# joelle-o-world/dusp

Hardware: AMD Instinct MI355X
Metric: rendered Msamples/sec (whole node) + HBM GB/s fraction, 1024-voice 48kHz (higher is better)
Workload: dtype f64; 1 GPU; configs[2] per-voice: 1024 voices/GPU x Multiply(Osc(10k), Ramp(T,1,0) triggered), 60s @48000 Hz, every voice's PCM written; voices_per_gpu=1024, voices_total=1024, n_samples=2880000, engine=fused, parallelism=voices sharded over 1 GPU(s), no collective

## Files before the change

### dusp_amd/csrc/abi_context.hip

```cpp
#include <cmath>
#include <cstdio>
#include <cstdlib>
#include <cstring>
#include <memory>

#include "abi_internal.hpp"
#include "device_util.hpp"
#include "jit_engine.hpp"
#include "table_checks.hpp"

thread_local std::string g_error;

static dusp::Knobs read_knobs() {
    dusp::Knobs k;
    auto num = [](const char *name, int fallback) {
        const char *e = getenv(name);
        return e && *e ? atoi(e) : fallback;
    };
    if (const char *t = getenv("DUSP_FUSED_TABLE")) k.fused_table_global = t[0] == 'g';
    k.fused_R = num("DUSP_FUSED_R", k.fused_R);
    k.fused_items = num("DUSP_FUSED_ITEMS", k.fused_items);
    k.fused_fx32 = num("DUSP_FUSED_FX32", k.fused_fx32);
    k.fused_segmajor = num("DUSP_FUSED_SEGMAJOR", k.fused_segmajor);
    k.wave_segments = num("DUSP_WAVE_SEGMENTS", k.wave_segments);
    k.wave_max_waves = num("DUSP_WAVE_MAX_WAVES", k.wave_max_waves);
    k.wave_jit = num("DUSP_WAVE_JIT", k.wave_jit);
    k.wave_per_wave = num("DUSP_WAVE_PER_WAVE", k.wave_per_wave);
    k.jit_profile = num("DUSP_JIT_PROFILE", k.jit_profile);
    k.filter_fma = num("DUSP_FILTER_FMA", k.filter_fma);
    k.jit_spill_bytes = num("DUSP_JIT_SPILL", k.jit_spill_bytes);
    k.jit_lds_table = num("DUSP_JIT_LDS_TABLE", k.jit_lds_table);
    k.jit_lean = num("DUSP_JIT_LEAN", k.jit_lean);
    k.jit_log = num("DUSP_JIT_LOG", k.jit_log);
    k.ring_window = num("DUSP_RING_WINDOW", k.ring_window);
    k.filter_scan = num("DUSP_FILTER_SCAN", k.filter_scan);
    k.filter_warm = num("DUSP_FILTER_WARM", k.filter_warm);
    k.jit_nt = num("DUSP_JIT_NT", k.jit_nt);
    k.delay_line = num("DUSP_DELAY_LINE", k.delay_line);
    k.jit_rotate = num("DUSP_JIT_ROTATE", k.jit_rotate);
    k.ring_poison = num("DUSP_RING_POISON", k.ring_poison);
    k.mix_width = num("DUSP_MIX_WIDTH", k.mix_width);
    k.mix_depth = num("DUSP_MIX_DEPTH", k.mix_depth);
    k.mix_tile_mb = num("DUSP_MIX_TILE_MB", k.mix_tile_mb);
    k.score_plan_kb = num("DUSP_SCORE_PLAN_KB", k.score_plan_kb);
    if (const char *f = getenv("DUSP_JIT_FORCE")) {
        int w = 0, r = 0;
        if (std::sscanf(f, "%dx%d", &w, &r) == 2 && w >= 1 && w <= 16 && r >= 1 && r <= 4) k.jit_force_waves = w, k.jit_force_per_wave = r;
    }
    return k;
}

extern "C" {

const char *dusp_version(void) { return "dusp-hip 0.1.0 (gfx950)"; }
int dusp_abi_version(void) { return DUSP_ABI_VERSION; }

// ... 197 lines not shown
```

### dusp_amd/csrc/abi_internal.hpp

```cpp
#pragma once
#include <limits>
#include <cmath>
#include <hip/hip_runtime.h>

#include <algorithm>
#include <cstddef>
#include <cstdint>
#include <exception>
#include <map>
#include <mutex>
#include <new>
#include <stdexcept>
#include <string>
#include <utility>
#include <vector>

#include "../../include/dusp_hip.h"
#include "device_types.hpp"
#include "fused_plan.hpp"
#include "jit_codegen.hpp"
#include "program.hpp"
#include "score_plan.hpp"

namespace dusp {
// ... 148 lines not shown
        f("staging parameters", d_host_par);
        f("staging inputs", d_host_in);
        f("hand-off buffers", d_handoff_init);
        f("hand-off buffers", d_handoff_out);
        f("program constants", d_ops);
        f("program constants", d_out_bufs);
        f("program constants", d_init);
        f("compiled kernel's constants", d_jit_fk);
        f("compiled kernel's constants", d_jit_dk);
        f("compiled kernel's constants", d_jit_scan);
        f("warm-up records", d_warm_records);
        f("warm-up start state", d_warm_init);
        f("column verdicts", d_jit_regime);
    }
    const char *first_overwritten() {
        const char *hit = nullptr;
        for_each_workspace([&](const char *name, auto &buf) {
            if (!hit && !buf.intact()) hit = name;
        });
        return hit;
    }
};
static_assert(sizeof(dusp_workspaces) == dusp_workspaces::kCount * sizeof(DevBuf<char>), "dusp_workspaces holds DevBufs only: update kCount and for_each_workspace");

struct dusp_program : dusp_workspaces {
    dusp_ctx *ctx = nullptr;
    dusp::Program P;
    int engine = DUSP_ENGINE_CHUNK;
    dusp::FusedPlan fused;
    dusp::WavePlan wave;
    std::vector<dusp::SumVoice> h_sum_voices;
    std::vector<double> h_sum_end;
    uint32_t last_n_inst = 0, last_n_pad = 0;
    bool rendered = false;
    std::vector<double> h_state;
    bool h_state_valid = false;
    bool mixed = false;
    std::vector<unsigned> mix_range;
    uint32_t mix_n_inst = 0;
    int requested_engine = DUSP_ENGINE_AUTO;
    bool resumable = false;
    bool persistent = false;
    bool keep_memory = false;
    bool delay_changed = false;
    bool migrate_to_chunk = false;
    int64_t next_clock = 0;
    hipEvent_t ev0 = nullptr, ev1 = nullptr;
    hipStream_t last_stream = nullptr;
    bool jit_ok = false;
    std::string jit_why;
    std::map<std::pair<int, int>, dusp::JitSource> jit_src;
    bool jit_consts_uploaded = false;
    int voice_loop = -1;
    uint64_t jit_table_generation = 0;
    int jit_waves = 0, jit_per_wave = 0;
    unsigned jit_segments = 1;
    unsigned wave_segments = 1;
    std::vector<double> param_bound;
    bool jit_voices = false;
    bool jit_scan = false;
    bool handoff_ok = false;
    std::string handoff_why;
    unsigned warm_redo_from = 0;
    unsigned char *pin[1] = {nullptr};
    size_t pin_bytes = 0;

// ... 135 lines not shown
```

### dusp_amd/csrc/abi_program.hip

```cpp
#include <cmath>
#include <cstdio>
#include <cstdlib>
#include <cstring>
#include <memory>

#include "abi_internal.hpp"
#include "engine_select.hpp"
#include "jit_engine.hpp"

extern "C" {

static int select_engine(dusp_program *prog) {
    dusp_ctx *ctx = prog->ctx;
    dusp::EngineRequest rq;
    rq.requested = prog->requested_engine;
    rq.resumable = prog->resumable;
    rq.rendered = prog->rendered;
    rq.engine_so_far = prog->engine;
    rq.delay_changed = prog->delay_changed;
    rq.wave_jit = ctx->knobs.wave_jit;
    for (int k = 0; k < dusp::kNumTables; k++) rq.table_set[k] = ctx->table_set[k], rq.table_fx32_ok[k] = ctx->table_fx32_ok[k];
    dusp::EngineChoice choice = dusp::engine_select(prog->P, rq, std::move(prog->wave.ramp_checked));
    prog->fused = std::move(choice.fused);
    prog->wave = std::move(choice.wave);
// ... 133 lines not shown
        prog->requested_engine = before.engine;
        const int back = finish_build(prog);
        prog->requested_engine = requested;
        ctx->err = back == DUSP_OK ? why : why + " (and the previous program could not be restored: " + ctx->err + ")";
        return rc;
    }
    prog->keep_memory = persistent;
    if (persistent && engine_before == DUSP_ENGINE_WAVE && prog->engine == DUSP_ENGINE_CHUNK) prog->migrate_to_chunk = true;
    return DUSP_OK;
    });
}

void dusp_program_destroy(dusp_program *prog) {
    if (!prog) return;
    (void)hipSetDevice(prog->ctx->device);
    if (prog->rendered && prog->ev1) (void)hipEventSynchronize(prog->ev1);
    (void)hipStreamSynchronize(prog->ctx->stream);
    delete prog;
}

int dusp_program_info_get(const dusp_program *prog, dusp_program_info *info) {
    if (!prog || !info) return DUSP_ERR_ARG;
    std::memset(info, 0, sizeof *info);
    const dusp::Graph &g = prog->P.g;
    info->sample_rate = (uint32_t)g.sample_rate;
    info->chunk_size = (uint32_t)g.chunk;
    info->n_units = (uint32_t)g.units.size();
    info->n_out_channels = (uint32_t)prog->P.out_bufs.size();
    info->n_params = (uint32_t)g.n_params;
    info->engine = (uint32_t)prog->engine;
    info->n_device_ops = (uint32_t)prog->P.ops.size();
    info->n_inputs = (uint32_t)g.n_inputs;
    if (prog->engine == DUSP_ENGINE_FUSED) std::snprintf(info->shape, sizeof info->shape, "%s", prog->fused.shape.c_str());
    if (prog->engine == DUSP_ENGINE_WAVE && prog->jit_ok && (prog->jit_waves || !prog->rendered))
    {
        const int at = std::snprintf(info->shape, sizeof info->shape, "%s, compiled kernel: %d units, %dx%d", prog->P.feed_forward ? "feed-forward" : "feedback",
                                     (int)prog->P.ops.size(), prog->jit_waves, prog->jit_per_wave);
        if (at > 0 && (size_t)at < sizeof info->shape && (prog->jit_voices || prog->jit_segments > 1)) {
            if (prog->jit_voices && prog->jit_segments > 1) std::snprintf(info->shape + at, sizeof info->shape - (size_t)at, ", loop, %u seg", prog->jit_segments);
            else if (prog->jit_voices) std::snprintf(info->shape + at, sizeof info->shape - (size_t)at, ", voice loop");
            else if (prog->warm_redo_from) std::snprintf(info->shape + at, sizeof info->shape - (size_t)at, ", %u seg, redo@%u", prog->jit_segments, prog->warm_redo_from);
            else std::snprintf(info->shape + at, sizeof info->shape - (size_t)at, ", %u seg", prog->jit_segments);
        } else if (at > 0 && (size_t)at < sizeof info->shape && prog->jit_scan)
            std::snprintf(info->shape + at, sizeof info->shape - (size_t)at, ", scan");
    }
    else if (prog->engine == DUSP_ENGINE_WAVE && prog->jit_ok)
        std::snprintf(info->shape, sizeof info->shape, "%s, %d chunk buffers in LDS (kernel compiling)", prog->P.feed_forward ? "feed-forward" : "feedback", prog->wave.n_slots);
    else if (prog->engine == DUSP_ENGINE_WAVE && prog->rendered && prog->wave_segments > 1)
        std::snprintf(info->shape, sizeof info->shape, "%s, %d chunk buffers in LDS, %u seg", prog->P.feed_forward ? "feed-forward" : "feedback", prog->wave.n_slots, prog->wave_segments);
    else if (prog->engine == DUSP_ENGINE_WAVE)
        std::snprintf(info->shape, sizeof info->shape, "%s, %d chunk buffers in LDS", prog->P.feed_forward ? "feed-forward" : "feedback", prog->wave.n_slots);
    if (prog->engine == DUSP_ENGINE_CHUNK && !prog->P.warm_ops.empty() && !prog->handoff_ok && !prog->handoff_why.empty())
        std::snprintf(info->shape, sizeof info->shape, "warm-up, then not compiled: %.34s", prog->handoff_why.c_str());
    if (prog->engine == DUSP_ENGINE_CHUNK && prog->handoff_ok && prog->jit_waves)
        std::snprintf(info->shape, sizeof info->shape, "%d warm-up chunks here, then compiled kernel: %d units, %dx%d", (int)prog->P.warm_ops.size(), (int)prog->P.ops.size(),
                      prog->jit_waves, prog->jit_per_wave);
    return DUSP_OK;
}

int dusp_state_download(dusp_program *prog, size_t instance, size_t unit, double *out, size_t cap) {
    if (!prog) return DUSP_ERR_ARG;
    dusp_ctx *ctx = prog->ctx;
    return guarded(ctx->err, "dusp_state_download", [&]() -> int {
    if (!prog->rendered) CTX_FAIL(ctx, DUSP_ERR_STATE, "dusp_state_download: nothing has been rendered yet");
    if (prog->mixed) CTX_FAIL(ctx, DUSP_ERR_STATE, "dusp_state_download: the last render was a mix (dusp_render_host_mix, dusp_render_host_score): unit state describes its last tile only");
    const dusp::Graph &g = prog->P.g;
// ... 138 lines not shown
```

### dusp_amd/csrc/abi_render.hip

```cpp
#include <cstring>

#include "abi_internal.hpp"
#include "jit_plan.hpp"
#include "render_plan.hpp"
#include "ring_windows.hpp"

static int check_tables(dusp_program *prog) {
    dusp_ctx *ctx = prog->ctx;
    for (const auto &u : prog->P.g.units)
        if (u.op == dusp::OP_OSC || u.op == dusp::OP_MULTI_OSC || u.op == dusp::OP_SHAPE) {
            const int w = (int)u.attrs[0];
            if (!ctx->d_tables || !ctx->table_set[w])
                CTX_FAIL(ctx, DUSP_ERR_STATE, "render: wave table " + std::to_string(w) + " has not been uploaded (dusp_table_upload)");
            if (ctx->table_len != (uint32_t)prog->P.g.sample_rate + 1)
                CTX_FAIL(ctx, DUSP_ERR_STATE, "render: wave table length != sample_rate + 1");
        }
    return DUSP_OK;
}


hipError_t zero_rings(dusp_program *prog, uint32_t n_pad, uint32_t n_chunks, bool instance_major, hipStream_t stream) {
    const dusp::Program &P = prog->P;
    float *rings = prog->d_rings.p;
    const size_t total = (size_t)P.ring_samples;
// ... 101 lines not shown
    }
    dusp::build_sum_voices(prog->fused, (uint32_t)prog->P.g.sample_rate, gb, L.chain_first + (uint64_t)c.n_chunks * dusp::kChunk, prog->h_sum_voices, prog->h_sum_end);
    HIP_TRY(ctx, prog->d_sum_voices.ensure(prog->h_sum_voices.size()));
    HIP_TRY(ctx, hipMemcpyAsync(prog->d_sum_voices.p, prog->h_sum_voices.data(), prog->h_sum_voices.size() * sizeof(dusp::SumVoice), hipMemcpyHostToDevice, stream));
    std::vector<double> end((size_t)prog->fused.n_state_words * n_inst);
    for (int w = 0; w < prog->fused.n_state_words; w++)
        for (uint32_t i = 0; i < n_inst; i++) end[(size_t)w * n_inst + i] = prog->h_sum_end[(size_t)w];
    HIP_TRY(ctx, hipMemcpyAsync(prog->d_fused_state.p, end.data(), end.size() * sizeof(double), hipMemcpyHostToDevice, stream));
    HIP_TRY(ctx, hipStreamSynchronize(stream));
    HIP_TRY(ctx, hipEventRecord(prog->ev0, stream));
    HIP_TRY(ctx, dusp::launch_sumchain(prog->fused, L, prog->d_sum_voices.p, gb, stream));
    HIP_TRY(ctx, hipEventRecord(prog->ev1, stream));
    return DUSP_OK;
}

static int render_fused(dusp_program *prog, const RenderCall &c, const ChainWindow *window) {
    dusp_ctx *ctx = prog->ctx;
    dusp::FusedLaunch L{};
    L.params = c.d_params;
    L.tables = ctx->d_tables;
    L.table_stride = ctx->table_stride;
    L.out = c.d_out;
    L.n_inst = c.n_inst;
    L.n_samples = c.n_samples;
    L.n_chunks = c.n_chunks;
    L.sample_rate = (uint32_t)prog->P.g.sample_rate;
    L.n_cus = ctx->n_cus;
    L.table_antisym = ctx->table_antisym[prog->fused.table_id];
    L.table_finite = ctx->table_finite[prog->fused.table_id];
    L.table_fx32_ok = ctx->table_fx32_ok[prog->fused.table_id];
    L.table_delta = ctx->table_delta[prog->fused.table_id];
    L.table_form = ctx->table_form[prog->fused.table_id];
    L.knobs = ctx->knobs;
    HIP_TRY(ctx, prog->d_recs.ensure(c.n_inst));
    L.recs = prog->d_recs.p;
    HIP_TRY(ctx, prog->d_fused_state.ensure((size_t)std::max(1, prog->fused.n_state_words) * c.n_inst));
    L.end_state = prog->d_fused_state.p;
    if (prog->fused.kind == dusp::FUSED_SUMCHAIN) {
        if (int rc = render_sum_chain(prog, c, L, window)) return rc;
    } else {
        HIP_TRY(ctx, hipEventRecord(prog->ev0, c.stream));
        HIP_TRY(ctx, dusp::launch_fused(prog->fused, L, c.stream));
        HIP_TRY(ctx, hipEventRecord(prog->ev1, c.stream));
    }
    finish_render(prog, c.n_inst, c.n_pad, c.n_chunks);
    return DUSP_OK;
}

static int render_wave_interpreter(dusp_program *prog, const RenderCall &c) {
    dusp_ctx *ctx = prog->ctx;
    const dusp::Program &P = prog->P;
    const uint32_t n_inst = c.n_inst, n_pad = c.n_pad, n_chunks = c.n_chunks;
    hipStream_t stream = c.stream;
    HIP_TRY(ctx, prog->d_state.ensure(state_workspace_doubles(P, n_pad)));
    dusp::WaveArgs w{};
    w.ops = prog->d_ops.p;
    w.out_bufs = prog->d_out_bufs.p;
    w.params = c.d_params;
    w.tables = ctx->d_tables;
    w.inputs = c.d_inputs;
    w.out = c.d_out;
    w.state = prog->d_state.p;
    w.init_state = prog->d_init.p;
    w.n_samples = c.n_samples;
    w.n_ops = (uint32_t)P.ops.size();
    w.n_out = (uint32_t)P.out_bufs.size();
    w.n_inst = n_inst;
// ... 202 lines not shown
```

### dusp_amd/csrc/device_types.hpp

```cpp
#pragma once
#if defined(__HIPCC_RTC__)
typedef unsigned int uint32_t;
typedef int int32_t;
typedef unsigned long long uint64_t;
typedef long long int64_t;
typedef unsigned long uintptr_t;
#else
#include <cstdint>
#endif

namespace dusp {

enum : int {
    OP_OSC = 1, OP_RAMP, OP_MULTIPLY, OP_SUM, OP_FILTER, OP_DELAY, OP_CB_READER, OP_CB_WRITER, OP_REPEATER,
    OP_SUBTRACT, OP_DIVIDE, OP_POLARITY_INVERT, OP_ABS, OP_CLIP, OP_HARD_CLIP_ABOVE, OP_HARD_CLIP_BELOW,
    OP_SECONDS_TO_SAMPLES, OP_FIXED_MULTIPLY, OP_GAIN, OP_DECIBEL_TO_SCALER, OP_SEMITONE_TO_RATIO, OP_POW,
    OP_FIXED_DELAY, OP_COMB_FILTER, OP_ALL_PASS, OP_MONO_DELAY, OP_READBACK_DELAY, OP_MULTI_OSC,
    OP_PAN, OP_MIDI_TO_FREQUENCY, OP_RESCALE, OP_CROSS_FADER, OP_VECTOR_MAGNITUDE, OP_TIMER, OP_SAMPLE_RATE_REDUX,
    OP_CONCAT_CHANNELS, OP_PICK_CHANNEL,
    OP_SHAPE, OP_AHD,
    OP_HOST_ONLY,
    OP_INPUT,
    OP_RETRIGGER,
    OP_MAP_FIRST = OP_SUBTRACT, OP_MAP_LAST = OP_POW,
    OP_WIDE_FIRST = OP_PAN, OP_WIDE_LAST = OP_VECTOR_MAGNITUDE
};
constexpr int kMaxIn = 5;
enum : int { IN_CONST = 0, IN_CONNECT = 1, IN_PARAM = 2 };
enum : int { SRC_CONST = 0, SRC_BUF = 1, SRC_PARAM = 2 };
constexpr int kNumTables = 9;
constexpr int kFirstShapeTable = 5;
constexpr int kChunk = 256;
constexpr unsigned long half_table_image_bytes(uint32_t sample_rate) {
    return ((unsigned long)((sample_rate / 2 + 1) + ((sample_rate / 2 + 1) >> 5) + 2) * 4ul + 15ul) & ~15ul;
}
constexpr int kMaxWarmChunks = 8;

struct Knobs {
    int fused_table_global = 0;
    int fused_R = 4;
    int fused_items = 0;
    int fused_fx32 = 1;
    int fused_segmajor = 0;
    int wave_segments = -1;
    int wave_max_waves = 0;
    int wave_jit = 1;
    int wave_per_wave = 0;
    int jit_lean = 1;
    int jit_log = 0;
    int jit_lds_table = 1;
    int jit_spill_bytes = 96;
    int jit_force_waves = 0;
    int jit_force_per_wave = 0;
    int ring_window = 1;
    int ring_poison = 0;
    int filter_scan = 1;
    int filter_warm = 1;
    int jit_nt = 0;
    int jit_rotate = 1;
    int delay_line = 1;
    int filter_fma = 0;
    int jit_profile = 0;
    int mix_width = 0;
    int mix_depth = 0;
    int mix_tile_mb = 0;
    int score_plan_kb = 0;
};

#if defined(__HIPCC__)
typedef float f32x4 __attribute__((ext_vector_type(4)));
#endif

struct DevOperand {
    int32_t kind;
    int32_t idx;
    float cval;
// ... 31 lines not shown
```

### dusp_amd/csrc/fused_engine.hip

```cpp
#include <hip/hip_runtime.h>

#include <type_traits>

#include "device_types.hpp"
#include "fused_device.hpp"
#include "fused_plan.hpp"
#include "repeat_add.hpp"

namespace dusp {

namespace {

template <bool FASTDIV>
__device__ __forceinline__ float ramp_value(const FusedArgs &A, double tn, double dy) {
    const double tt = fmin(tn, A.r_d);
    double q;
    if (FASTDIV) {
        q = tt * A.r_rcp;
        const double rem = fma(-q, A.r_d, tt);
        q = fma(rem, A.r_rcp, q);
    } else
        q = tt / A.r_d;
    return (float)(A.r_y0 + q * dy);
}

__device__ __forceinline__ float shape_value(const FusedArgs &A, double t, double srd) {
    const double l = (double)A.s_min, h = (double)A.s_max;
    if (t <= 0.0) return (float)((A.s_left_is_shape ? (double)A.s_table[0] : A.s_left) * (h - l) + l);
    if (t > srd) return (float)((A.s_right_is_shape ? (double)A.s_table[(uint32_t)srd] : A.s_right) * (h - l) + l);
    if (t != t) return __builtin_nanf("");
    const double fl = floor(t), frac = t - fl;
    return (float)(l + (h - l) * ((double)A.s_table[(int)ceil(t)] * frac + (double)A.s_table[(int)fl] * (1.0 - frac)));
}

__device__ __forceinline__ void start_phase(const OscRec &rc, uint32_t seg, uint32_t lane, uint64_t (&P)[4]) {
    const uint64_t base = addmod(addmod(rc.P0, rc.Fm, rc.S), mulmod(rc.segstep, seg, rc.S), rc.S);
    P[0] = addmod(base, mulmod(rc.step4, lane, rc.S), rc.S);
    for (int c = 1; c < 4; ++c) P[c] = addmod(P[c - 1], rc.Fm, rc.S);
}

}

static __device__ int fused_prepare_voice(const FusedArgs &A, OscRec *recs, const uint32_t inst) {
    const uint32_t sr = A.sample_rate;
    const double srd = (double)sr;
    OscRec rc;
    double fd = (double)operand_value(A.f, A.params, A.n_inst, inst);
    const float f_in = operand_value(A.f, A.params, A.n_inst, inst);
    rc.bad = !(fabs(fd) <= 3.4028234663852886e38);
    if (!rc.bad && osc_const_beyond_exact(f_in, sr)) rc.bad = 2;
    if (rc.bad) fd = 0.0;
    if (fabs(fd) >= srd) fd = fmod(fd, srd);
    int E = 0;
    if (fd != 0.0) E = min(E, lsb_exponent(fd));
    if (A.phase0 != 0.0) E = min(E, lsb_exponent(A.phase0));
    const int Emin = -(62 - (32 - __builtin_clz(sr)));
    if (E < Emin) E = Emin;
    rc.E = E;
    rc.u = ldexp(1.0, E);
    rc.S = (uint64_t)sr << (-E);
    const long long F = (long long)rint(ldexp(fd, -E));
    rc.Fm = F >= 0 ? (uint64_t)F : rc.S - (uint64_t)(-F);
    if (rc.Fm >= rc.S) rc.Fm -= rc.S;
    rc.P0 = (uint64_t)rint(ldexp(A.phase0, -E));
    if (rc.P0 >= rc.S) rc.P0 %= rc.S;
    rc.step4 = mulmod(rc.Fm, 4, rc.S);
    rc.step256 = mulmod(rc.Fm, kChunk, rc.S);
    rc.segstep = mulmod(rc.Fm, (uint64_t)A.seg_groups * kChunk, rc.S);
    rc.gain = A.gain.kind == SRC_PARAM || A.gain.kind == SRC_CONST ? operand_value(A.gain, A.params, A.n_inst, inst) : 1.f;
    rc.pad = 0;
    recs[inst] = rc;
// ... 16 lines not shown
        const double t_end = A.s_playing ? repeat_add(A.s_t0, A.s_c, T_end) : A.s_t0;
        A.end_state[(size_t)A.shape_state_word * A.n_inst + inst] = t_end;
        A.end_state[(size_t)(A.shape_state_word + 1) * A.n_inst + inst] = A.s_playing ? 1.0 : 0.0;
        A.end_state[(size_t)(A.shape_state_word + 2) * A.n_inst + inst] = (A.s_finished || (T_end > 0 && t_end > srd)) ? 1.0 : 0.0;
    }
    return rc.bad;
}

static __device__ void fused_reference_voice(const FusedArgs &A, const OscRec *recs, const uint32_t inst, const uint32_t lane, const int kind) {
    const double srd = (double)A.sample_rate, dy = A.r_y1 - A.r_y0;
    const float f = operand_value(A.f, A.params, A.n_inst, inst), gain = recs[inst].gain;
    float *row = A.out + (size_t)inst * A.n_samples;
    double phase = A.phase0;
    for (uint32_t g = 0; g < A.n_groups; ++g) {
        double mine[4];
        phase = osc_reference_chunk(phase, srd, lane, [&](uint32_t, int) { return f; }, mine);
#pragma unroll
        for (int c = 0; c < 4; ++c) {
            const uint64_t n = (uint64_t)g * kChunk + lane * 4 + c;
            float v = osc_reference_lookup(A.table, mine[c], srd);
            if (kind == FUSED_OSC_RAMP) v = v * ramp_value<false>(A, A.r_playing ? A.r_t0 + (double)(n + 1) : A.r_t0, dy);
            if (kind == FUSED_OSC_SHAPE) v = v * shape_value(A, A.s_playing ? repeat_add(A.s_t0, A.s_c, n + 1) : A.s_t0, srd);
            if (kind == FUSED_OSC_GAIN) v = v * gain;
            if (n < A.n_samples) row[n] = fix_out<false>(v);
        }
    }
}

__global__ void __launch_bounds__(256) dusp_fused_prepare(FusedArgs A, OscRec *recs, int kind) {
    __shared__ uint32_t flagged[256], n_flagged;
    if (threadIdx.x == 0) n_flagged = 0u;
    __syncthreads();
    const uint32_t inst = blockIdx.x * blockDim.x + threadIdx.x;
    if (inst < A.n_inst && fused_prepare_voice(A, recs, inst) == 2) flagged[atomicAdd(&n_flagged, 1u)] = inst;
    __syncthreads();
    for (uint32_t k = threadIdx.x >> 6; k < n_flagged; k += 4u) fused_reference_voice(A, recs, flagged[k], threadIdx.x & 63u, kind);
}

template <int KIND, int TBL, int R, bool FASTDIV, bool FINITE, int BLOCK>
__global__ void __launch_bounds__(BLOCK) dusp_fused_kernel(FusedArgs A, const OscRec *__restrict__ recs) {
    extern __shared__ __attribute__((aligned(16))) float lds_table[];
    Table<TBL> table;
    table.g = A.table;
    table.h = lds_table;
    table.N = A.sample_rate + 1;
    table.M = A.sample_rate / 2;
    table.form = make_table_form(A.table_form, A.sample_rate);
    if (TBL == 1) load_half_table<BLOCK>(lds_table, A.table, A.sample_rate);
    const uint32_t lane = threadIdx.x & 63u;
    constexpr uint32_t waves_per_block = BLOCK / 64;
    constexpr int RS = R < 4 ? R : 4;
    const uint32_t n_blk = (A.n_inst + R - 1) / R;
    const uint64_t n_items = (uint64_t)n_blk * A.n_seg;
    const uint64_t total_waves = (uint64_t)gridDim.x * waves_per_block;
    const double srd = (double)A.sample_rate;
    const uint32_t sr = A.sample_rate;
    const double dy = A.r_y1 - A.r_y0;
    const uint32_t n_full = A.vec4_ok ? (uint32_t)(A.n_samples / kChunk) : 0u;

    for (uint64_t item = (uint64_t)blockIdx.x * waves_per_block + (threadIdx.x >> 6); item < n_items; item += total_waves) {
        const uint32_t blk = A.seg_major ? (uint32_t)(item / A.n_seg) : (uint32_t)(item % n_blk);
        const uint32_t seg = A.seg_major ? (uint32_t)(item % A.n_seg) : (uint32_t)(item / n_blk);
        const uint32_t g0 = seg * A.seg_groups;
        const uint32_t g1 = min(g0 + A.seg_groups, A.n_groups);
        const uint32_t gm = max(g0, min(g1, n_full));
        const uint64_t t_start = (uint64_t)g0 * kChunk;

        uint32_t inst[R];
        int e_min = 0;
        bool any_bad = false;
#pragma unroll
        for (int r = 0; r < R; ++r) {
            inst[r] = min(blk * R + r, A.n_inst - 1);
            e_min = min(e_min, recs[inst[r]].E);
            any_bad = any_bad || recs[inst[r]].bad;
        }
        float *const row0 = A.out + t_start + lane * 4;
        const double tn0 = A.r_t0 + (A.r_playing ? (double)(t_start + lane * 4 + 1) : 0.0);
        const double tn_step = A.r_playing ? (double)kChunk : 0.0;
        const double tn_c = A.r_playing ? 1.0 : 0.0;
        double tn;
        const double st0 = (KIND == FUSED_OSC_SHAPE && A.s_playing) ? repeat_add(A.s_t0, A.s_c, t_start) : A.s_t0;
        double st;
        auto ramp4 = [&](float (&rv)[4]) {
            if (KIND == FUSED_OSC_SHAPE) {
                if (!A.s_playing) {
#pragma unroll
                    for (int c = 0; c < 4; ++c) rv[c] = shape_value(A, st, srd);
                } else {
                    long long T, ce;
                    int K;
                    if (linear_run(st, A.s_c, kChunk, T, ce, K)) {
                        T += (long long)(lane * 4) * ce;
#pragma unroll
                        for (int c = 0; c < 4; ++c) {
                            T += ce;
                            rv[c] = shape_value(A, ldexp((double)T, K - 52), srd);
                        }
                        st = ldexp((double)(T + (long long)(kChunk - 4 - lane * 4) * ce), K - 52);
                    } else {
                        double t = repeat_add(st, A.s_c, (uint64_t)lane * 4);
#pragma unroll
                        for (int c = 0; c < 4; ++c) rv[c] = shape_value(A, t = t + A.s_c, srd);
                        st = __shfl(t, 63, 64);
                    }
                }
            }
            if (KIND == FUSED_OSC_RAMP) {
                rv[0] = ramp_value<FASTDIV>(A, tn, dy);
#pragma unroll
                for (int c = 1; c < 4; ++c) rv[c] = ramp_value<FASTDIV>(A, tn + tn_c * c, dy);
                tn += tn_step;
            }
        };
        auto finish = [&](float v, float rv, float gain) {
            if (KIND == FUSED_OSC_RAMP || KIND == FUSED_OSC_SHAPE) v = v * rv;
            if (KIND == FUSED_OSC_GAIN) v = v * gain;
            return fix_out<FINITE>(v);
        };

        if (e_min == 0 && !any_bad) {
            uint32_t idx[R][4], step[R];
            size_t roff[R];
            float gain[R];
#pragma unroll
            for (int r = 0; r < R; ++r) {
                const OscRec rc = recs[inst[r]];
                uint64_t P[4];
                start_phase(rc, seg, lane, P);
                for (int c = 0; c < 4; ++c) idx[r][c] = (uint32_t)P[c];
                step[r] = (uint32_t)rc.step256;
                roff[r] = (size_t)inst[r] * A.n_samples;
                gain[r] = rc.gain;
            }
            tn = tn0;
            st = st0;
            float *row = row0;
            auto run = [&](uint32_t ga, uint32_t gb, auto vec) {
                for (uint32_t g = ga; g < gb; ++g) {
                    float rv[4] = {1.f, 1.f, 1.f, 1.f};
                    ramp4(rv);
#pragma unroll
                    for (int r = 0; r < R; ++r) {
                        float v[4];
#pragma unroll
                        for (int c = 0; c < 4; ++c) {
                            v[c] = finish(table.at(idx[r][c]), rv[c], gain[r]);
                            idx[r][c] += step[r];
                            idx[r][c] = min(idx[r][c], idx[r][c] - sr);
                        }
                        store4<decltype(vec)::value>(row + roff[r], v, (uint64_t)g * kChunk + lane * 4, A.n_samples);
                    }
// ... 166 lines not shown
            st = st0;
                float *row = row0;
                auto run = [&](uint32_t ga, uint32_t gb, auto vec) {
                    for (uint32_t g = ga; g < gb; ++g) {
                        float rv[4] = {1.f, 1.f, 1.f, 1.f};
                        ramp4(rv);
#pragma unroll
                        for (int r = 0; r < RS; ++r) {
                            float v[4];
#pragma unroll
                            for (int c = 0; c < 4; ++c) {
                                const uint32_t idx = (uint32_t)(int)ph[r][c];
                                const double fraction = ph[r][c] - (double)(int)idx;
                                float ta, tb;
                                table.pair(idx, ta, tb);
                                float x = (float)((double)ta * (1.0 - fraction) + (double)tb * fraction);
                                if (bad[r]) x = 0.f;
                                v[c] = finish(x, rv[c], gain[r]);
                                ph[r][c] += D[r];
                                if (ph[r][c] >= srd) ph[r][c] -= srd;
                            }
                            if (bad[r] != 2) store4<decltype(vec)::value>(row + roff[r], v, (uint64_t)g * kChunk + lane * 4, A.n_samples);
                        }
                        row += kChunk;
                    }
                };
                run(g0, gm, std::true_type{});
                run(gm, g1, std::false_type{});
            }
        }
    }
}

template <int KIND, int TBL, int R, bool FASTDIV, bool FINITE, int BLOCK>
static hipError_t launch_one(const FusedArgs &A, const OscRec *recs, int grid, size_t lds_bytes, hipStream_t stream) {
    auto kernel = dusp_fused_kernel<KIND, TBL, R, FASTDIV, FINITE, BLOCK>;
    if (lds_bytes > 65536) {
        hipError_t e = hipFuncSetAttribute((const void *)kernel, hipFuncAttributeMaxDynamicSharedMemorySize, (int)lds_bytes);
        if (e != hipSuccess) return e;
    }
    hipLaunchKernelGGL(kernel, dim3((unsigned)grid), dim3(BLOCK), lds_bytes, stream, A, recs);
    return hipGetLastError();
}

hipError_t launch_fused(const FusedPlan &plan, const FusedLaunch &L, hipStream_t stream) {
    FusedArgs A{};
    A.params = L.params;
    A.table = L.tables + (size_t)plan.table_id * L.table_stride;
    A.out = L.out;
    A.end_state = L.end_state;
    A.n_samples = L.n_samples;
    A.n_inst = L.n_inst;
    A.n_groups = (uint32_t)((L.n_samples + kChunk - 1) / kChunk);
    A.sample_rate = L.sample_rate;
    A.n_chunks = L.n_chunks;
    A.f = plan.f;
    A.gain = plan.gain;
    if (plan.kind != FUSED_OSC_GAIN) A.gain.kind = -1;
    A.phase0 = plan.phase0;
    A.r_d = plan.r_d; A.r_y0 = plan.r_y0; A.r_y1 = plan.r_y1; A.r_t0 = plan.r_t0; A.r_rcp = plan.r_rcp;
    A.r_playing = plan.r_playing;
    A.r_fastdiv = plan.r_fastdiv;
    A.vec4_ok = (L.n_samples % 4 == 0) && (((uintptr_t)L.out & 15) == 0);
    A.osc_state_word = 0;
    A.ramp_state_word = plan.kind == FUSED_OSC_RAMP ? 1 : -1;
    A.shape_state_word = plan.kind == FUSED_OSC_SHAPE ? 1 : -1;
    if (plan.kind == FUSED_OSC_SHAPE) {
        A.s_table = L.tables + (size_t)plan.s_table_id * L.table_stride;
        A.s_t0 = plan.s_t0; A.s_c = plan.s_c; A.s_min = plan.s_min; A.s_max = plan.s_max;
        A.s_left = plan.s_left; A.s_right = plan.s_right;
        A.s_left_is_shape = plan.s_left_is_shape; A.s_right_is_shape = plan.s_right_is_shape;
        A.s_playing = plan.s_playing; A.s_finished = plan.s_finished;
    }
    auto ordinary = [](double y) { return y == 0.0 || (std::fabs(y) >= 9.3e-10 && std::fabs(y) <= 1.1e18); };
    A.r_scale_ok = plan.kind == FUSED_OSC_RAMP && ordinary(plan.r_y0) && ordinary(plan.r_y1) && plan.r_d <= 1.1e12 && (plan.r_t0 == 0.0 || plan.r_t0 >= 1.0) &&
                           L.knobs.fused_fx32 != 2
                       ? 1 : 0;
    A.fx32_ok = L.table_fx32_ok && L.knobs.fused_fx32 ? 1 : 0;
    A.table_delta = L.knobs.fused_fx32 == 1 ? L.table_delta : 0;
    A.seg_major = L.knobs.fused_segmajor;

    int tbl = (L.table_antisym && L.sample_rate % 2 == 0) ? 1 : 0;
    if (L.table_form >= TABLE_FORM_SAW && L.table_form <= TABLE_FORM_TRIANGLE) tbl = 2;
    A.table_form = L.table_form;
    if (L.knobs.fused_table_global) tbl = 0;
    const size_t lds_bytes = tbl == 1 ? half_table_lds_bytes(L.sample_rate) : 0;
    if (lds_bytes > 160 * 1024) tbl = 0;

    int R = L.knobs.fused_R;
    if (R != 1 && R != 4 && R != 8) R = 4;
    const int block = tbl == 1 ? 1024 : 256;
    const int grid = tbl == 1 ? L.n_cus : L.n_cus * 8;
    const uint64_t total_waves = (uint64_t)grid * (block / 64);
    const uint64_t n_blk = (A.n_inst + R - 1) / R;
    auto cut = [&](uint64_t per_wave, uint64_t &n_seg) {
        n_seg = std::max<uint64_t>(1, (total_waves * per_wave + n_blk - 1) / n_blk);
        return (A.n_groups + n_seg - 1) / n_seg;
    };
    uint64_t n_seg = 1, seg = 0;
    if (L.knobs.fused_items > 0) seg = cut((uint64_t)L.knobs.fused_items, n_seg);
    else if ((seg = cut(4, n_seg)) < 64) seg = cut(2, n_seg);
    if (seg < 16) seg = 16;
    if (seg > 4096) seg = 4096;
    A.seg_groups = (uint32_t)seg;
    A.n_seg = (A.n_groups + A.seg_groups - 1) / A.seg_groups;
    const bool finite = L.table_finite && plan.kind != FUSED_OSC_GAIN && std::isfinite(plan.r_y0) && std::isfinite(plan.r_y1);

    hipLaunchKernelGGL(dusp_fused_prepare, dim3((A.n_inst + 255) / 256), dim3(256), 0, stream, A, L.recs, (int)plan.kind);
    hipError_t e = hipGetLastError();
    if (e != hipSuccess) return e;

    auto render = [&]() -> hipError_t {
#define DUSP_L3(KIND, RR, FD, FIN) \
    return tbl == 1 ? launch_one<KIND, 1, RR, FD, FIN, 1024>(A, L.recs, grid, lds_bytes, stream) \
                    : launch_one<KIND, 0, RR, FD, FIN, 256>(A, L.recs, grid, 0, stream)
#define DUSP_L2(KIND, FD, FIN) \
    do { if (tbl == 2) return launch_one<KIND, 2, 4, FD, FIN, 256>(A, L.recs, grid, 0, stream); \
         if (R == 8) { DUSP_L3(KIND, 8, FD, FIN); } if (R == 4) { DUSP_L3(KIND, 4, FD, FIN); } DUSP_L3(KIND, 1, FD, FIN); } while (0)
    switch (plan.kind) {
    case FUSED_OSC:
        if (finite) DUSP_L2(FUSED_OSC, false, true);
        DUSP_L2(FUSED_OSC, false, false);
    case FUSED_OSC_RAMP:
        if (plan.r_fastdiv && finite) DUSP_L2(FUSED_OSC_RAMP, true, true);
        if (plan.r_fastdiv) DUSP_L2(FUSED_OSC_RAMP, true, false);
        DUSP_L2(FUSED_OSC_RAMP, false, false);
    case FUSED_OSC_GAIN: DUSP_L2(FUSED_OSC_GAIN, false, false);
    case FUSED_OSC_SHAPE: DUSP_L2(FUSED_OSC_SHAPE, false, false);
    }
#undef DUSP_L2
#undef DUSP_L3
        return hipErrorInvalidValue;
    };
    return render();
}

}
```

### dusp_amd/csrc/fused_plan.hpp

```cpp
#pragma once
#include <algorithm>
#include <cmath>
#include <limits>
#include <string>
#include <vector>

#include "device_types.hpp"
#include "program.hpp"

namespace dusp {

enum : int { FUSED_OSC = 0, FUSED_OSC_RAMP = 1, FUSED_OSC_GAIN = 2, FUSED_SUMCHAIN = 3, FUSED_OSC_SHAPE = 4 };

struct FusedPlan {
    std::string shape, why;
    int kind = FUSED_OSC;
    int table_id = 0;
    DevOperand f{}, gain{};
    double phase0 = 0;
    double r_d = 1, r_y0 = 0, r_y1 = 0, r_t0 = 0, r_rcp = 1;
    int r_playing = 0, r_fastdiv = 0;
    int s_table_id = 0, s_playing = 0, s_finished = 0, s_left_is_shape = 0, s_right_is_shape = 0;
    double s_t0 = 0, s_c = 0, s_left = 0, s_right = 0;
    float s_min = 0, s_max = 1;
// ... 74 lines not shown
    std::vector<int> order;
    std::vector<int> buf_slot;
    std::vector<int> op_state;
    int n_slots = 0, n_state_ops = 0;
    int ext_units = 0;
    bool ring_events = false;
    bool splittable = false;
    bool splittable_but_for_filters = false;
    int max_osc_level = 0;
    std::vector<int> osc_level;
    std::vector<int> ramp_fastdiv;
    struct RampChecked { double d, t0; bool ok; };
    std::vector<RampChecked> ramp_checked;
    int lds_table_id = -1;
    std::string why;
};

struct FusedLaunch {
    const float *params;
    const float *tables;
    float *out;
    double *end_state;
    OscRec *recs;
    uint64_t n_samples;
    uint32_t n_inst, n_chunks, sample_rate, table_stride;
    int n_cus;
    bool table_antisym, table_finite, table_fx32_ok;
    const float *chain_init = nullptr;
    uint64_t chain_first = 0;
    bool chain_raw = false;
    int table_delta;
    int table_form;
    Knobs knobs;
};

struct FusedArgs {
    const float *params;
    const float *table;
    float *out;
    double *end_state;
    uint64_t n_samples;
    uint32_t n_inst, n_groups, seg_groups, n_seg, sample_rate, n_chunks;
    DevOperand f, gain;
    double phase0;
    double r_d, r_y0, r_y1, r_t0, r_rcp;
    int32_t r_playing, r_fastdiv, vec4_ok, osc_state_word, ramp_state_word, fx32_ok, seg_major, r_scale_ok;
    const float *s_table;
    double s_t0, s_c, s_left, s_right;
    float s_min, s_max;
    int32_t s_playing, s_finished, shape_state_word, s_left_is_shape, s_right_is_shape;
    int32_t table_form;
    int32_t table_delta;
};

inline bool ramp_fastdiv_ok(double t0, double d, bool playing) {
    const double r = 1.0 / d;
    auto same = [&](double t) {
        const double q = t * r;
        const double rem = std::fma(-q, d, t);
        return std::fma(rem, r, q) == t / d;
    };
    if (!same(t0) || !same(d)) return false;
    if (!playing) return true;
    const double steps = std::ceil(d - t0) + 1;
    if (!(steps < 67108864.0)) return false;
    double t = t0;
    for (long k = 0; k < (long)steps; k++) {
        t += 1.0;
        if (t > d) break;
        if (!same(t)) return false;
    }
    return true;
}

inline bool plan_fused(const Program &P, FusedPlan &plan) {
    const Graph &g = P.g;
    auto no = [&](const std::string &why) {
        plan.why = why;
        return false;
    };
    if (!P.warm_ops.empty()) return no("channel counts grow during the first chunks");
    if (!P.feed_forward) return no("feedback edge");
    if (!g.rings.empty() || P.ring_samples) return no("rings");
    if (P.out_bufs.size() != 1) return no("multichannel output");
    for (const auto &u : g.units)
        if (u.n_out != 1) return no("multichannel unit");
// ... 524 lines not shown
```

Before: 1.317 million Msamples/s.

## Reuse per-period oscillator table values across sample-rate periods in fused kernel

Adds a periodic rendering path for fused oscillator kernels. When every voice's phase is exactly integral per second (checked on device in the prepare kernel via per-block flags), each wave computes table lookups for one window once and replays them for every one-second period, recomputing only the ramp or gain. The aim is to cut table lookups and modular phase arithmetic, leaving mostly stores. The cost is a device-side flag scan at kernel start, more register pressure from the cached values, and a different work distribution across waves.

```diff
diff --git a/dusp_amd/csrc/abi_context.hip b/dusp_amd/csrc/abi_context.hip
--- a/dusp_amd/csrc/abi_context.hip
+++ b/dusp_amd/csrc/abi_context.hip
@@ -22,6 +22,8 @@
     k.fused_items = num("DUSP_FUSED_ITEMS", k.fused_items);
     k.fused_fx32 = num("DUSP_FUSED_FX32", k.fused_fx32);
     k.fused_segmajor = num("DUSP_FUSED_SEGMAJOR", k.fused_segmajor);
+    k.fused_periodic = num("DUSP_FUSED_PERIODIC", k.fused_periodic);
+    k.fused_periodic_m = num("DUSP_FUSED_PERIODIC_M", k.fused_periodic_m);
     k.wave_segments = num("DUSP_WAVE_SEGMENTS", k.wave_segments);
     k.wave_max_waves = num("DUSP_WAVE_MAX_WAVES", k.wave_max_waves);
     k.wave_jit = num("DUSP_WAVE_JIT", k.wave_jit);
diff --git a/dusp_amd/csrc/abi_internal.hpp b/dusp_amd/csrc/abi_internal.hpp
--- a/dusp_amd/csrc/abi_internal.hpp
+++ b/dusp_amd/csrc/abi_internal.hpp
@@ -204,6 +204,8 @@
     std::vector<dusp::SumVoice> h_sum_voices;
     std::vector<double> h_sum_end;
     uint32_t last_n_inst = 0, last_n_pad = 0;
+    int32_t fused_item_shape[3] = {0, 0, 0};
+    uint32_t fused_item_n_inst = 0;
     bool rendered = false;
     std::vector<double> h_state;
     bool h_state_valid = false;
diff --git a/dusp_amd/csrc/abi_program.hip b/dusp_amd/csrc/abi_program.hip
--- a/dusp_amd/csrc/abi_program.hip
+++ b/dusp_amd/csrc/abi_program.hip
@@ -189,6 +189,14 @@
     info->n_device_ops = (uint32_t)prog->P.ops.size();
     info->n_inputs = (uint32_t)g.n_inputs;
     if (prog->engine == DUSP_ENGINE_FUSED) std::snprintf(info->shape, sizeof info->shape, "%s", prog->fused.shape.c_str());
+    if (prog->engine == DUSP_ENGINE_FUSED && prog->rendered && prog->fused_item_shape[0] && prog->d_recs.p && prog->ev1) {
+        std::vector<uint32_t> off_int(((size_t)prog->fused_item_n_inst + 255) / 256, 1u);
+        bool all_int = hipSetDevice(prog->ctx->device) == hipSuccess && hipEventSynchronize(prog->ev1) == hipSuccess &&
+                       hipMemcpy(off_int.data(), prog->d_recs.p + prog->fused_item_n_inst, off_int.size() * sizeof(uint32_t), hipMemcpyDeviceToHost) == hipSuccess;
+        for (uint32_t w : off_int) all_int = all_int && w == 0u;
+        const size_t at = std::strlen(info->shape);
+        if (all_int) std::snprintf(info->shape + at, sizeof info->shape - at, ", periodic items %dx%d", (int)prog->fused_item_shape[1], (int)prog->fused_item_shape[2]);
+    }
     if (prog->engine == DUSP_ENGINE_WAVE && prog->jit_ok && (prog->jit_waves || !prog->rendered))
     {
         const int at = std::snprintf(info->shape, sizeof info->shape, "%s, compiled kernel: %d units, %dx%d", prog->P.feed_forward ? "feed-forward" : "feedback",
diff --git a/dusp_amd/csrc/abi_render.hip b/dusp_amd/csrc/abi_render.hip
--- a/dusp_amd/csrc/abi_render.hip
+++ b/dusp_amd/csrc/abi_render.hip
@@ -157,7 +157,10 @@
     L.table_delta = ctx->table_delta[prog->fused.table_id];
     L.table_form = ctx->table_form[prog->fused.table_id];
     L.knobs = ctx->knobs;
-    HIP_TRY(ctx, prog->d_recs.ensure(c.n_inst));
+    prog->fused_item_shape[0] = 0;
+    L.item_shape = prog->fused_item_shape;
+    prog->fused_item_n_inst = c.n_inst;
+    HIP_TRY(ctx, prog->d_recs.ensure(dusp::fused_recs_needed(c.n_inst)));
     L.recs = prog->d_recs.p;
     HIP_TRY(ctx, prog->d_fused_state.ensure((size_t)std::max(1, prog->fused.n_state_words) * c.n_inst));
     L.end_state = prog->d_fused_state.p;
diff --git a/dusp_amd/csrc/device_types.hpp b/dusp_amd/csrc/device_types.hpp
--- a/dusp_amd/csrc/device_types.hpp
+++ b/dusp_amd/csrc/device_types.hpp
@@ -42,6 +42,8 @@
     int fused_items = 0;
     int fused_fx32 = 1;
     int fused_segmajor = 0;
+    int fused_periodic = 1;
+    int fused_periodic_m = 0;
     int wave_segments = -1;
     int wave_max_waves = 0;
     int wave_jit = 1;
diff --git a/dusp_amd/csrc/fused_engine.hip b/dusp_amd/csrc/fused_engine.hip
--- a/dusp_amd/csrc/fused_engine.hip
+++ b/dusp_amd/csrc/fused_engine.hip
@@ -37,6 +37,80 @@
     const uint64_t base = addmod(addmod(rc.P0, rc.Fm, rc.S), mulmod(rc.segstep, seg, rc.S), rc.S);
     P[0] = addmod(base, mulmod(rc.step4, lane, rc.S), rc.S);
     for (int c = 1; c < 4; ++c) P[c] = addmod(P[c - 1], rc.Fm, rc.S);
+}
+
+template <int KIND, bool FINITE>
+__device__ __forceinline__ float finish_sample(float v, float rv, float gain) {
+    if (KIND == FUSED_OSC_RAMP || KIND == FUSED_OSC_SHAPE) v = v * rv;
+    if (KIND == FUSED_OSC_GAIN) v = v * gain;
+    return fix_out<FINITE>(v);
+}
+
+template <int KIND, int TBL, int R, int M, bool FASTDIV, bool FINITE>
+__device__ __forceinline__ void fused_periodic_items(const FusedArgs &A, const OscRec *__restrict__ recs, const Table<TBL> &table, const uint32_t wave,
+                                                     const uint32_t total_waves) {
+    const uint32_t lane = threadIdx.x & 63u;
+    const uint32_t sr = A.sample_rate;
+    const uint32_t n_blk = (A.n_inst + R - 1) / R;
+    const uint32_t n_items = n_blk * A.p_windows;
+    const double dy = A.r_y1 - A.r_y0;
+    const double tn_c = A.r_playing ? 1.0 : 0.0, tn_step = A.r_playing ? (double)kChunk : 0.0, tn_period = A.r_playing ? (double)sr : 0.0;
+    for (uint32_t item = wave; item < n_items; item += total_waves) {
+        const uint32_t blk = A.seg_major ? item / A.p_windows : item % n_blk;
+        const uint32_t win = A.seg_major ? item % A.p_windows : item / n_blk;
+        const uint32_t s0 = win * M;
+        const uint32_t q0 = s0 * kChunk + lane * 4;
+        float val[R][M][4], gain[R];
+        size_t roff[R];
+#pragma unroll
+        for (int r = 0; r < R; ++r) {
+            const uint32_t inst = min(blk * R + r, A.n_inst - 1);
+            const OscRec rc = recs[inst];
+            uint64_t P = addmod(addmod(addmod(rc.P0, rc.Fm, rc.S), mulmod(rc.step256, s0, rc.S), rc.S), mulmod(rc.step4, lane, rc.S), rc.S);
+#pragma unroll
+            for (int j = 0; j < M; ++j) {
+                uint64_t Pc = P;
+#pragma unroll
+                for (int c = 0; c < 4; ++c) {
+                    val[r][j][c] = table.at((uint32_t)Pc);
+                    Pc = addmod(Pc, rc.Fm, rc.S);
+                }
+                P = addmod(P, rc.step256, rc.S);
+            }
+            roff[r] = (size_t)inst * A.n_samples;
+            gain[r] = rc.gain;
+        }
+        const bool whole = (s0 + M) * kChunk <= sr;
+        double tn = A.r_t0 + (A.r_playing ? (double)(q0 + 1) : 0.0);
+        auto period = [&](const uint64_t base, auto guarded) {
+            double t = tn;
+#pragma unroll
+            for (int j = 0; j < M; ++j) {
+                float rv[4] = {1.f, 1.f, 1.f, 1.f};
+                if (KIND == FUSED_OSC_RAMP) {
+                    rv[0] = ramp_value<FASTDIV>(A, t, dy);
+#pragma unroll
+                    for (int c = 1; c < 4; ++c) rv[c] = ramp_value<FASTDIV>(A, t + tn_c * c, dy);
+                    t += tn_step;
+                }
+                const uint32_t q = q0 + j * kChunk;
+                const bool live = !decltype(guarded)::value || (q < sr && base + q < A.n_samples);
+#pragma unroll
+                for (int r = 0; r < R; ++r) {
+                    float v[4];
+#pragma unroll
+                    for (int c = 0; c < 4; ++c) v[c] = finish_sample<KIND, FINITE>(val[r][j][c], rv[c], gain[r]);
+                    if (live) store4<true>(A.out + (roff[r] + base) + q, v, 0, 0);
+                }
+            }
+        };
+        const uint64_t w0 = (uint64_t)s0 * kChunk, w1 = w0 + (uint64_t)M * kChunk;
+        for (uint64_t base = 0; base + w0 < A.n_samples; base += sr) {
+            if (whole && base + w1 <= A.n_samples) period(base, std::false_type{});
+            else period(base, std::true_type{});
+            tn += tn_period;
+        }
+    }
 }
 
 }
@@ -119,12 +193,18 @@
     if (threadIdx.x == 0) n_flagged = 0u;
     __syncthreads();
     const uint32_t inst = blockIdx.x * blockDim.x + threadIdx.x;
-    if (inst < A.n_inst && fused_prepare_voice(A, recs, inst) == 2) flagged[atomicAdd(&n_flagged, 1u)] = inst;
-    __syncthreads();
+    int off_int = 0;
+    if (inst < A.n_inst) {
+        const int bad = fused_prepare_voice(A, recs, inst);
+        if (bad == 2) flagged[atomicAdd(&n_flagged, 1u)] = inst;
+        off_int = bad != 0 || recs[inst].E != 0;
+    }
+    const int any_off_int = __syncthreads_or(off_int);
+    if (threadIdx.x == 0) ((uint32_t *)(recs + A.n_inst))[blockIdx.x] = any_off_int ? 1u : 0u;
     for (uint32_t k = threadIdx.x >> 6; k < n_flagged; k += 4u) fused_reference_voice(A, recs, flagged[k], threadIdx.x & 63u, kind);
 }
 
-template <int KIND, int TBL, int R, bool FASTDIV, bool FINITE, int BLOCK>
+template <int KIND, int TBL, int R, bool FASTDIV, bool FINITE, int BLOCK, bool PERIODIC>
 __global__ void __launch_bounds__(BLOCK) dusp_fused_kernel(FusedArgs A, const OscRec *__restrict__ recs) {
     extern __shared__ __attribute__((aligned(16))) float lds_table[];
     Table<TBL> table;
@@ -145,6 +225,20 @@
     const double dy = A.r_y1 - A.r_y0;
     const uint32_t n_full = A.vec4_ok ? (uint32_t)(A.n_samples / kChunk) : 0u;
 
+    if (PERIODIC && KIND != FUSED_OSC_SHAPE && A.periodic_ok) {
+        const uint32_t *off_int = (const uint32_t *)(recs + A.n_inst);
+        uint32_t any = 0u;
+        for (uint32_t k = lane; k < (A.n_inst + 255u) / 256u; k += 64u) any |= off_int[k];
+        if (__builtin_amdgcn_ballot_w64(any != 0u) == 0ull) {
+            const uint32_t wave = (uint32_t)__builtin_amdgcn_readfirstlane((int)(blockIdx.x * waves_per_block + (threadIdx.x >> 6)));
+            const uint32_t waves = gridDim.x * waves_per_block;
+            if (R * 4 * 4 <= 64 && A.p_m == 4) fused_periodic_items<KIND, TBL, R, (R * 4 * 4 <= 64 ? 4 : 2), FASTDIV, FINITE>(A, recs, table, wave, waves);
+            else if (R * 3 * 4 <= 64 && A.p_m == 3) fused_periodic_items<KIND, TBL, R, (R * 3 * 4 <= 64 ? 3 : 2), FASTDIV, FINITE>(A, recs, table, wave, waves);
+            else fused_periodic_items<KIND, TBL, R, 2, FASTDIV, FINITE>(A, recs, table, wave, waves);
+            return;
+        }
+    }
+
     for (uint64_t item = (uint64_t)blockIdx.x * waves_per_block + (threadIdx.x >> 6); item < n_items; item += total_waves) {
         const uint32_t blk = A.seg_major ? (uint32_t)(item / A.n_seg) : (uint32_t)(item % n_blk);
         const uint32_t seg = A.seg_major ? (uint32_t)(item % A.n_seg) : (uint32_t)(item / n_blk);
@@ -200,11 +294,7 @@
                 tn += tn_step;
             }
         };
-        auto finish = [&](float v, float rv, float gain) {
-            if (KIND == FUSED_OSC_RAMP || KIND == FUSED_OSC_SHAPE) v = v * rv;
-            if (KIND == FUSED_OSC_GAIN) v = v * gain;
-            return fix_out<FINITE>(v);
-        };
+        auto finish = [&](float v, float rv, float gain) { return finish_sample<KIND, FINITE>(v, rv, gain); };
 
         if (e_min == 0 && !any_bad) {
             uint32_t idx[R][4], step[R];
@@ -437,15 +527,21 @@
     }
 }
 
-template <int KIND, int TBL, int R, bool FASTDIV, bool FINITE, int BLOCK>
-static hipError_t launch_one(const FusedArgs &A, const OscRec *recs, int grid, size_t lds_bytes, hipStream_t stream) {
-    auto kernel = dusp_fused_kernel<KIND, TBL, R, FASTDIV, FINITE, BLOCK>;
+template <int KIND, int TBL, int R, bool FASTDIV, bool FINITE, int BLOCK, bool PERIODIC>
+static hipError_t launch_variant(const FusedArgs &A, const OscRec *recs, int grid, size_t lds_bytes, hipStream_t stream) {
+    auto kernel = dusp_fused_kernel<KIND, TBL, R, FASTDIV, FINITE, BLOCK, PERIODIC>;
     if (lds_bytes > 65536) {
         hipError_t e = hipFuncSetAttribute((const void *)kernel, hipFuncAttributeMaxDynamicSharedMemorySize, (int)lds_bytes);
         if (e != hipSuccess) return e;
     }
     hipLaunchKernelGGL(kernel, dim3((unsigned)grid), dim3(BLOCK), lds_bytes, stream, A, recs);
     return hipGetLastError();
+}
+
+template <int KIND, int TBL, int R, bool FASTDIV, bool FINITE, int BLOCK>
+static hipError_t launch_one(const FusedArgs &A, const OscRec *recs, int grid, size_t lds_bytes, hipStream_t stream) {
+    if (A.periodic_ok) return launch_variant<KIND, TBL, R, FASTDIV, FINITE, BLOCK, KIND != FUSED_OSC_SHAPE>(A, recs, grid, lds_bytes, stream);
+    return launch_variant<KIND, TBL, R, FASTDIV, FINITE, BLOCK, false>(A, recs, grid, lds_bytes, stream);
 }
 
 hipError_t launch_fused(const FusedPlan &plan, const FusedLaunch &L, hipStream_t stream) {
@@ -509,6 +605,8 @@
     if (seg > 4096) seg = 4096;
     A.seg_groups = (uint32_t)seg;
     A.n_seg = (A.n_groups + A.seg_groups - 1) / A.seg_groups;
+    plan_periodic(A, plan.kind, tbl == 2 ? 4 : R, total_waves, L.knobs.fused_periodic, L.knobs.fused_periodic_m);
+    if (L.item_shape) L.item_shape[0] = A.periodic_ok, L.item_shape[1] = tbl == 2 ? 4 : R, L.item_shape[2] = A.p_m;
     const bool finite = L.table_finite && plan.kind != FUSED_OSC_GAIN && std::isfinite(plan.r_y0) && std::isfinite(plan.r_y1);
 
     hipLaunchKernelGGL(dusp_fused_prepare, dim3((A.n_inst + 255) / 256), dim3(256), 0, stream, A, L.recs, (int)plan.kind);
diff --git a/dusp_amd/csrc/fused_plan.hpp b/dusp_amd/csrc/fused_plan.hpp
--- a/dusp_amd/csrc/fused_plan.hpp
+++ b/dusp_amd/csrc/fused_plan.hpp
@@ -130,6 +130,7 @@
     int table_delta;
     int table_form;
     Knobs knobs;
+    int32_t *item_shape = nullptr;
 };
 
 struct FusedArgs {
@@ -149,7 +150,51 @@
     int32_t s_playing, s_finished, shape_state_word, s_left_is_shape, s_right_is_shape;
     int32_t table_form;
     int32_t table_delta;
+    int32_t periodic_ok;
+    int32_t p_m;
+    uint32_t p_windows;
 };
+
+inline size_t fused_recs_needed(size_t n_inst) {
+    const size_t flag_bytes = ((n_inst + 255) / 256) * sizeof(uint32_t);
+    return n_inst + (flag_bytes + sizeof(OscRec) - 1) / sizeof(OscRec);
+}
+
+constexpr int kPeriodicMinPeriods = 8;
+inline bool plan_periodic(FusedArgs &A, int kind, int R, uint64_t total_waves, int mode, int force_m) {
+    A.periodic_ok = 0;
+    A.p_m = 2;
+    A.p_windows = 1;
+    if (mode <= 0) return false;
+    if (kind != FUSED_OSC && kind != FUSED_OSC_RAMP && kind != FUSED_OSC_GAIN) return false;
+    const uint64_t sr = A.sample_rate;
+    if (sr < 4 || sr % 4 != 0 || !A.vec4_ok) return false;
+    if (kind == FUSED_OSC_RAMP && !(A.r_t0 == std::floor(A.r_t0) && std::fabs(A.r_t0) < 9007199254740992.0 && A.r_t0 + (double)A.n_samples < 9007199254740992.0))
+        return false;
+    if (A.n_samples < sr * (uint64_t)(mode >= 2 ? 1 : kPeriodicMinPeriods)) return false;
+    const uint64_t steps = (sr + kChunk - 1) / kChunk, n_blk = (A.n_inst + (uint64_t)R - 1) / (uint64_t)R;
+    if (n_blk * ((steps + 1) / 2) + total_waves >= (1ull << 31)) return false;
+    const bool forced = force_m >= 2 && force_m <= 4 && R * force_m * 4 <= 64;
+    uint64_t best = 0;
+    for (int m = 2; m <= 4; m++) {
+        if (R * m * 4 > 64 || (forced && m != force_m)) continue;
+        const uint64_t windows = (steps + (uint64_t)m - 1) / (uint64_t)m;
+        const uint64_t dealt = ((n_blk * windows + total_waves - 1) / total_waves) * (uint64_t)m;
+        if (!best || dealt <= best) {
+            best = dealt;
+            A.p_m = m;
+            A.p_windows = (uint32_t)windows;
+        }
+    }
+    if (mode == 1) {
+        if (sr < 4096) return false;
+        const uint64_t periods = (A.n_samples + sr - 1) / sr;
+        const uint64_t even = (n_blk * A.n_groups + total_waves - 1) / total_waves;
+        if (best * periods * 8 > even * 9) return false;
+    }
+    A.periodic_ok = 1;
+    return true;
+}
 
 inline bool ramp_fastdiv_ok(double t0, double d, bool playing) {
     const double r = 1.0 / d;
```

Result: faster. 1.359 million Msamples/s (median of 6 runs) (+3.1%).
